# rakhimovv/lvt

Measured on AMD Instinct MI355X. Metric: video-clips/sec/node (VQVAE+DSFVT train step, BAIR 64x64x16), higher is better.
Workload: dtype f32

## Files before the change

### include/lvt_hip.h

```cpp
#ifndef LVT_HIP_H
#define LVT_HIP_H
#include <stddef.h>
#include <stdint.h>
#ifdef __cplusplus
extern "C" {
#endif

#define LVT_OK            0
#define LVT_EINVAL      (-1)
#define LVT_EWORKSPACE  (-2)
#define LVT_ELAUNCH     (-3)
#define LVT_ENODEVICE   (-4)

const char *lvt_last_error(void);
int lvt_version(void);
int lvt_device_info(char *name, int name_len, int *cus, int *clock_khz, long long *hbm_bytes);

#define LVT_MATH_F32   (1 << 16)
#define LVT_MATH_F16X2 (1 << 18)
typedef struct { const float *a; const float *b; float *c; } lvt_amax_io;
int lvt_amax(const float *x, long long n, float *out, void *stream);
typedef struct { const float *x; long long n; float *out; } lvt_amax_entry;
int lvt_amax_multi(const lvt_amax_entry *entries, int n, void *stream);
int lvt_amax_merge(const float *a, const float *b, float *out, void *stream);
// ... 23 lines not shown
    const float *B; long long ldb; int b_kb; long long b_skb;
    float *C;       long long ldc;
    int batch_outer, batch_inner;
    long long sA_o, sA_i, sB_o, sB_i, sC_o, sC_i;
    float alpha;
    int flags;
    const float *bias;
    const float *res;  long long ldr;
    const float *mask; long long ldm;
    int splits;
    float *a_colsum;
    long long c_plane;
    const float *a_amax, *b_amax;
    const float *a_amax2, *b_amax2;
    float *c_amax;
} lvt_gemm_desc;
size_t lvt_gemm_workspace_bytes(const lvt_gemm_desc *d);
int lvt_gemm_f32(const lvt_gemm_desc *d, void *workspace, size_t workspace_bytes, void *stream);

int lvt_vq_argmax_scores(const float *scores, long long rows, int K, long long ld, const float *codebook, int D,
                         long long *idx, void *stream);

typedef struct {
    int M, N, K;
    const void *A; long long lda; int a_planes; int a_kb; long long a_skb;
    const void *B; long long ldb;
    float *C; long long ldc;
    int batch_outer, batch_inner;
    long long sA_o, sA_i, sB_o, sB_i, sC_o, sC_i;
    float alpha;
// ... 113 lines not shown
                     const float *g2_dev, const float *G, float *out, float *out_amax, void *stream);
int lvt_l1_bwd_plus(const float *a, const float *b, long long n, double denom, float scale, const float *gout_dev,
                    const float *g2_dev, const float *G, float *out, float *out_amax, void *stream);
int lvt_tanh_bwd(const float *g, const float *y, long long n, float *out, float *out_amax, void *stream);
int lvt_sigmoid_bwd(const float *g, const float *y, long long n, float *out, float *out_amax, void *stream);
int lvt_axpy(const float *x, const float *add, long long n, const float *alpha_dev, float alpha,
             float *out, void *stream);
int lvt_add_periodic(float *x, const float *table, long long rows, int P, int d, void *stream);

int lvt_layernorm_fwd(const float *x, long long rows, int d, float eps, const float *w, const float *b,
                      float *y, float *mean, float *rstd, float *y_amax, const float *w_amax, const float *b_amax,
                      void *stream);
int lvt_layernorm_fwd_p2(const float *x, long long rows, int d, float eps, const float *w, const float *b,
                         float *y, void *yp, float *mean, float *rstd, float *y_amax, const float *w_amax,
                         const float *b_amax, void *stream);
size_t lvt_layernorm_bwd_workspace_bytes(int d);
int lvt_layernorm_bwd(const float *dy, const float *x, const float *mean, const float *rstd,
                      const float *w, long long rows, int d, const float *add, float *dx, float *dw,
                      float *db, float *dx_amax, void *workspace, size_t workspace_bytes, void *stream);

int lvt_attn_softmax_fwd(float *scores, int B, int H, int S, float temper, const float *dt,
                         const float *dh, const float *dw, int bt, int bh, int bw, int masked, float fill,
                         void *stream);
int lvt_attn_softmax_bwd(const float *P, float *dP, int B, int H, int S, float temper, int bt, int bh,
                         int bw, float *G, float *ddt, float *ddh, float *ddw, void *stream);

int lvt_attn_fwd(const float *q, const float *k, const float *v, int B, int H, int S, int da, float temper,
                 const float *dt, const float *dh, const float *dw, int bt, int bh, int bw, int masked, float fill,
                 float *P, float *o, void *stream);

// ... 154 lines not shown
```

### lvt_amd/csrc/elementwise.hip

```cpp
#include "lvt_common.h"

static inline int grid_for(long long n, int per_block, int cap = 8192) {
    long long b = lvt_cdiv(n, per_block);
    if (b < 1) b = 1;
    return (int)(b < cap ? b : cap);
}

__device__ __forceinline__ float wave_sum(float v) {
#pragma unroll
    for (int off = 32; off >= 1; off >>= 1) v += __shfl_xor(v, off);
    return v;
}
__device__ __forceinline__ float wave_max(float v) {
#pragma unroll
    for (int off = 32; off >= 1; off >>= 1) v = fmaxf(v, __shfl_xor(v, off));
    return v;
}

__global__ void lvt_to_channels_last_kernel(const float *__restrict__ in, int B, int C, long long R, int ldo,
                                            int mode, const float *__restrict__ a, const float *__restrict__ s,
                                            float *__restrict__ out, float *__restrict__ out_amax) {
    __shared__ float amax_scratch[4];
    float am = 0.f;
    const long long total = (long long)B * R * ldo;
// ... 326 lines not shown
                const float a0 = v[i].x - mean, a1 = v[i].y - mean, a2 = v[i].z - mean, a3 = v[i].w - mean;
                q += (a0 * a0 + a1 * a1) + (a2 * a2 + a3 * a3);
            }
        }
        const float rstd = 1.0f / sqrtf(wave_sum(q) / d + eps);
        float4 *yp = reinterpret_cast<float4 *>(y + row * d);
#pragma unroll
        for (int i = 0; i < LN_MAXV; ++i) {
            const int c = lane + 64 * i;
            if (c < d4) {
                const float4 ww = reinterpret_cast<const float4 *>(w)[c];
                const float4 bb = reinterpret_cast<const float4 *>(b)[c];
                float4 o;
                o.x = (v[i].x - mean) * rstd * ww.x + bb.x; o.y = (v[i].y - mean) * rstd * ww.y + bb.y;
                o.z = (v[i].z - mean) * rstd * ww.z + bb.z; o.w = (v[i].w - mean) * rstd * ww.w + bb.w;
                yp[c] = o;
                if (P2) {
                    uint2 ph, pl;
                    ln_split_pair(o.x, o.y, ps, ph.x, pl.x);
                    ln_split_pair(o.z, o.w, ps, ph.y, pl.y);
                    char *ip = yimg + (long long)row * d * 4 + (c >> 3) * 128 + (c & 7) * 8;
                    *reinterpret_cast<uint2 *>(ip) = ph;
                    *reinterpret_cast<uint2 *>(ip + 64) = pl;
                }
                am = fmaxf(am, fmaxf(fmaxf(lvt_absf(o.x), lvt_absf(o.y)), fmaxf(lvt_absf(o.z), lvt_absf(o.w))));
            }
        }
        if (lane == 0 && mean_out) { mean_out[row] = mean; rstd_out[row] = rstd; }
    }
    if (y_amax) lvt_block_amax_commit(am, y_amax, amax_scratch);
}
// ... 5 lines not shown
    LVT_REQUIRE(!w_amax == !b_amax, "layernorm_fwd: w_amax and b_amax come together");
    hipLaunchKernelGGL(lvt_layernorm_fwd_kernel<0>, dim3(grid_for(rows, 4, (y_amax && !w_amax) ? 2048 : LN_FWD_MAX_BLOCKS)), dim3(256), 0,
                       (hipStream_t)stream, x, rows, d, eps, w, b, y, mean, rstd, y_amax, w_amax, b_amax, (char *)nullptr);
    LVT_CHECK_LAUNCH("lvt_layernorm_fwd_kernel");
    return LVT_OK;
}
extern "C" int lvt_layernorm_fwd_p2(const float *x, long long rows, int d, float eps, const float *w, const float *b,
                                    float *y, void *yp, float *mean, float *rstd, float *y_amax, const float *w_amax,
                                    const float *b_amax, void *stream) {
    LVT_REQUIRE(x && w && b && y && yp && rows > 0 && d % 32 == 0 && d <= 256 * LN_MAXV, "layernorm_fwd_p2: bad args (d=%d)", d);
    LVT_REQUIRE(y_amax && w_amax && b_amax, "layernorm_fwd_p2: the image is scaled by the a-priori bound: y_amax, w_amax, b_amax are required");
    LVT_REQUIRE(((uintptr_t)yp & 127) == 0, "layernorm_fwd_p2: the image must be 128-byte aligned");
    hipLaunchKernelGGL(lvt_layernorm_fwd_kernel<1>, dim3(grid_for(rows, 4, LN_FWD_MAX_BLOCKS)), dim3(256), 0,
                       (hipStream_t)stream, x, rows, d, eps, w, b, y, mean, rstd, y_amax, w_amax, b_amax, (char *)yp);
    LVT_CHECK_LAUNCH("lvt_layernorm_fwd_kernel<p2>");
    return LVT_OK;
}

#define LN_BWD_BLOCKS 512
#define LN_BWD_ROWS 1
__global__ __launch_bounds__(256) void lvt_layernorm_bwd_kernel(
    const float *__restrict__ dy, const float *__restrict__ x, const float *__restrict__ mean,
    const float *__restrict__ rstd, const float *__restrict__ w, long long rows, int d, const float *__restrict__ add,
    float *__restrict__ dx, float *__restrict__ pdw, float *__restrict__ pdb, float *__restrict__ dx_amax) {
    __shared__ float amax_scratch[4];
    float am = 0.f;
    __shared__ float sdw[4][256 * LN_MAXV];
    __shared__ float sdb[4][256 * LN_MAXV];
    const int lane = threadIdx.x & 63, wave = threadIdx.x >> 6;
    const int d4 = d / 4;
// ... 280 lines not shown
```

### lvt_amd/csrc/gemm_engine.hip

```cpp
#include "lvt_common.h"
#include "epilogue_fast.h"
#include <string.h>
#include <stdlib.h>
#include <stdint.h>
#include <type_traits>

typedef float f32x16 __attribute__((ext_vector_type(16)));

#define BK 32
#define NTHREADS 256

enum { A_KPLAIN = 0, A_MPLAIN = 1, A_CONV_K = 2, A_CONVT_K = 3, A_CONV_M = 4, A_ONEHOT_M = 5, A_PATCH = 6, A_PATCHT = 7 };
enum { B_KPLAIN = 0, B_NPLAIN = 1, B_CONVT_W = 2 };

struct KParams {
    int M, N, K;
    const float *A; long long lda; int a_kb; long long a_skb;
    const float *B; long long ldb; int b_kb; long long b_skb;
    float *C; long long ldc; long long c_plane;
    int batch_inner;
    long long sA_o, sA_i, sB_o, sB_i, sC_o, sC_i;
    float alpha; int flags;
    const float *bias; const float *res; long long ldr; const float *mask; long long ldm;
    int splits; int k_per_split; float *partial; long long partial_stride;
    int vec_epi;
    float *colsum_partial;
    const float *a_amax, *b_amax;
    const float *a_amax2, *b_amax2;
    float *c_amax;
    lvt_conv_geom g;
    const char *b_img;
    int Tq, Hq, Wq;
    int jT, jH, jW;
    const long long *oh_idx; long long oh_bstride, oh_pstride; int oh_P, oh_V; int oh_off[32];
};

__device__ __forceinline__ float4 ldg4(const float *p) { return *reinterpret_cast<const float4 *>(p); }

__device__ __forceinline__ unsigned cvt_pk_bf16(float lo, float hi) {
    unsigned r;
    asm("v_cvt_pk_bf16_f32 %0, %1, %2" : "=v"(r) : "v"(lo), "v"(hi));
    return r;
}
__device__ __forceinline__ float bf_lo(unsigned p) { return __uint_as_float(p << 16); }
// ... 1267 lines not shown
    else lvt_epilogue_vec<A_PATCHT, BM, BN, WM, WN>(p, acc, lds, m0, n0, wm, wn, lane, phase, 0, 0, 0);
}

#define WIDE_THREADS 512
#define WT_PA (256 + 32)
#define WT_PB (128 + 32)
typedef short s16x4 __attribute__((ext_vector_type(4)));
__device__ __forceinline__ f16x8 wide_tr_frag(const unsigned short *p, int pitch4) {
    typedef __attribute__((address_space(3))) s16x4 lds_v4;
    const s16x4 lo = __builtin_amdgcn_ds_read_tr16_b64_v4i16((lds_v4 *)(p));
    const s16x4 hi = __builtin_amdgcn_ds_read_tr16_b64_v4i16((lds_v4 *)(p + pitch4));
    union { struct { s16x4 a, b; } s; f16x8 v; } u;
    u.s.a = lo; u.s.b = hi;
    return u.v;
}
template <int TA, int TB>
__global__ __launch_bounds__(WIDE_THREADS, 2) void lvt_gemm_wide_kernel(const KParams p) {
    constexpr int BM = 256, BN = 128, WM = 4, WN = 2, TM = 2, TN = 2;
    constexpr int AMODE = TA ? A_MPLAIN : A_KPLAIN;
    constexpr int PA = WT_PA, PB = WT_PB;
    constexpr int PSA = TA ? BK * PA : HPlane<BM>::SIZE, PSB = TB ? BK * PB : HPlane<BN>::SIZE;
    constexpr int STAGE = 2 * (PSA + PSB);
    static_assert(PA % 4 == 0 && PB % 4 == 0 && PSA % 8 == 0 && PSB % 8 == 0, "transposing reads need 8-byte aligned addresses");
    static_assert(BK * PA <= HPlane<BM>::SIZE && BK * PB <= HPlane<BN>::SIZE, "the memory-order images are the smaller ones");
    constexpr int STAGE_FLOATS = (2 * STAGE) / 2 + 8;
    constexpr int TURN_FLOATS = WM * WN * 32 * (TN * 32);
    constexpr int LDS_FLOATS = STAGE_FLOATS > TURN_FLOATS ? STAGE_FLOATS : TURN_FLOATS;
    __shared__ __attribute__((aligned(16))) float lds[LDS_FLOATS];
    unsigned short *S0 = reinterpret_cast<unsigned short *>(lds);

    const int tid = threadIdx.x, lane = tid & 63, wave = tid >> 6;
    const int wm = wave / WN, wn = wave % WN;
// ... 5 lines not shown
    const float sa = lvt_f16_scale(p.a_amax, unscale, p.a_amax2), sb = lvt_f16_scale(p.b_amax, unscale, p.b_amax2);

    float4 av[4], bv[2];
    const int r0 = tid >> 3, kq = tid & 7;
    const int kk0 = TA ? tid >> 6 : 0, mq = tid & 63;
    const int bkk0 = tid >> 5, bnq = tid & 31;
    const char *Ak = reinterpret_cast<const char *>(tc.A), *Bk = reinterpret_cast<const char *>(tc.B);
    unsigned aoff[4], boff_g[2];
    int a_kin = 0, b_kin = 0;
    if (!TA) {
#pragma unroll
        for (int i = 0; i < 4; ++i) aoff[i] = (unsigned)(((long long)min(m0 + r0 + 64 * i, p.M - 1) * p.lda + kq * 4) * 4);
        const int blk = kbeg / p.a_kb;
        a_kin = kbeg - blk * p.a_kb;
        Ak += ((long long)blk * p.a_skb + a_kin) * 4;
    } else {
        const int m = m0 + mq * 4;
#pragma unroll
        for (int i = 0; i < 4; ++i) aoff[i] = (unsigned)(((long long)(kk0 * 4 + i) * p.lda + (m < p.M ? m : 0)) * 4);
        Ak += (long long)kbeg * p.lda * 4;
    }
    if (!TB) {
#pragma unroll
        for (int i = 0; i < 2; ++i) boff_g[i] = (unsigned)(((long long)min(n0 + r0 + 64 * i, p.N - 1) * p.ldb + kq * 4) * 4);
        const int blk = kbeg / p.b_kb;
        b_kin = kbeg - blk * p.b_kb;
        Bk += ((long long)blk * p.b_skb + b_kin) * 4;
    } else {
        const int n = n0 + bnq * 4;
#pragma unroll
        for (int i = 0; i < 2; ++i) boff_g[i] = (unsigned)(((long long)(bkk0 * 2 + i) * p.ldb + (n < p.N ? n : 0)) * 4);
        Bk += (long long)kbeg * p.ldb * 4;
    }
    const bool sum_on = TA && p.colsum_partial != nullptr && n0 == 0;
    float4 colacc = zero4();
    auto fetch = [&]() {
#pragma unroll
        for (int i = 0; i < 4; ++i) av[i] = *reinterpret_cast<const float4 *>(Ak + aoff[i]);
        if (!TA) {
            a_kin += BK;
            const bool wrap = a_kin >= p.a_kb;
            Ak += wrap ? ((long long)p.a_skb - p.a_kb + BK) * 4 : (long long)BK * 4;
            a_kin = wrap ? 0 : a_kin;
        } else {
            Ak += (long long)BK * p.lda * 4;
            if (sum_on) {
#pragma unroll
                for (int i = 0; i < 4; ++i) { colacc.x += av[i].x; colacc.y += av[i].y; colacc.z += av[i].z; colacc.w += av[i].w; }
            }
// ... 4 lines not shown
            b_kin += BK;
            const bool wrap = b_kin >= p.b_kb;
            Bk += wrap ? ((long long)p.b_skb - p.b_kb + BK) * 4 : (long long)BK * 4;
            b_kin = wrap ? 0 : b_kin;
        } else {
#pragma unroll
            for (int i = 0; i < 2; ++i) bv[i] = *reinterpret_cast<const float4 *>(Bk + boff_g[i]);
            Bk += (long long)BK * p.ldb * 4;
        }
    };
    auto store = [&](unsigned short *buf) {
        unsigned short *Ah = buf, *Bh = buf + 2 * PSA;
        if (!TA) {
#pragma unroll
            for (int i = 0; i < 4; ++i) store_split2_k<BM>(Ah, r0 + 64 * i, kq * 4, av[i], sa);
        } else {
#pragma unroll
            for (int i = 0; i < 4; ++i) {
                uint2 ph, pl;
                split2(av[i], sa, ph, pl);
                unsigned short *d = Ah + (kk0 * 4 + i) * PA + mq * 4;
                *reinterpret_cast<uint2 *>(d) = ph;
                *reinterpret_cast<uint2 *>(d + PSA) = pl;
            }
        }
        if (!TB) {
#pragma unroll
            for (int i = 0; i < 2; ++i) store_split2_k<BN>(Bh, r0 + 64 * i, kq * 4, bv[i], sb);
        } else {
#pragma unroll
// ... 318 lines not shown
    }
    if ((p.flags & LVT_EPI_PLANES) && !pv.vec_epi) {
        lvt_set_error("gemm: LVT_EPI_PLANES needs 16-byte aligned bias / res / mask and ldr, ldm %% 4 == 0");
        return LVT_EINVAL;
    }
    if (math_of(p.flags) == 2)
        hipLaunchKernelGGL((lvt_gemm_kernel<AMODE, BMODE, BM, BN, WM, WN, 2>), grid, dim3(NTHREADS), 0, s, pv);
    else if (math_of(p.flags) == 1)
        hipLaunchKernelGGL((lvt_gemm_kernel<AMODE, BMODE, BM, BN, WM, WN, 1>), grid, dim3(NTHREADS), 0, s, pv);
    else
        hipLaunchKernelGGL((lvt_gemm_kernel<AMODE, BMODE, BM, BN, WM, WN, 0>), grid, dim3(NTHREADS), 0, s, pv);
    LVT_CHECK_LAUNCH("lvt_gemm_kernel");
    return LVT_OK;
}

template <int TA, int TB>
static int launch_wide(const KParams &p, int zcount, hipStream_t s) {
    const long long ntm = lvt_cdiv(p.M, 256), ntn = lvt_cdiv(p.N, 128);
    if (ntm * ntn > 0x7fffffffLL || zcount > 65535 || p.splits > 65535) {
        lvt_set_error("gemm: grid too large (%lld tiles, z=%d, splits=%d)", ntm * ntn, zcount, p.splits);
        return LVT_EINVAL;
    }
    dim3 grid((unsigned)(ntm * ntn), (unsigned)zcount, (unsigned)(p.splits > 1 ? p.splits : 1));
    KParams pv = p;
    {
        auto al16 = [](const void *q) { return ((uintptr_t)q & 15) == 0; };
        bool ok = p.N % 4 == 0;
        if (p.splits > 1) ok = ok && al16(p.partial) && p.partial_stride % 4 == 0 && ((long long)p.M * p.N) % 4 == 0;
        else {
            ok = ok && al16(p.C) && p.ldc % 4 == 0 && p.sC_o % 4 == 0 && p.sC_i % 4 == 0;
            if (p.flags & LVT_EPI_BIAS) ok = ok && al16(p.bias);
            if (p.flags & LVT_EPI_RESIDUAL) ok = ok && al16(p.res) && p.ldr % 4 == 0;
            if (p.flags & LVT_EPI_MASK) ok = ok && al16(p.mask) && p.ldm % 4 == 0;
        }
        pv.vec_epi = ok ? 1 : 0;
    }
    if ((p.flags & LVT_EPI_PLANES) && !pv.vec_epi) {
        lvt_set_error("gemm: LVT_EPI_PLANES needs 16-byte aligned bias / res / mask and ldr, ldm %% 4 == 0");
        return LVT_EINVAL;
    }
    hipLaunchKernelGGL((lvt_gemm_wide_kernel<TA, TB>), grid, dim3(WIDE_THREADS), 0, s, pv);
    LVT_CHECK_LAUNCH("lvt_gemm_wide_kernel");
    return LVT_OK;
}

static int choose_splits(long long tiles, int K, int min_k) {
    int s = (int)((2 * LVT_NUM_CU) / (tiles > 0 ? tiles : 1));
    const int maxs = K / min_k > 0 ? K / min_k : 1;
    if (s > maxs) s = maxs;
    if (s < 1) s = 1;
    return s;
}

static void kparams_from_desc(const lvt_gemm_desc *d, KParams &p) {
    memset(&p, 0, sizeof(p));
    p.M = d->M; p.N = d->N; p.K = d->K;
    p.A = d->A; p.lda = d->lda; p.a_kb = d->a_kb > 0 ? d->a_kb : d->K; p.a_skb = d->a_skb;
    p.B = d->B; p.ldb = d->ldb; p.b_kb = d->b_kb > 0 ? d->b_kb : d->K; p.b_skb = d->b_skb;
    p.C = d->C; p.ldc = d->ldc; p.c_plane = d->c_plane;
    p.batch_inner = d->batch_inner > 0 ? d->batch_inner : 1;
    p.sA_o = d->sA_o; p.sA_i = d->sA_i; p.sB_o = d->sB_o; p.sB_i = d->sB_i; p.sC_o = d->sC_o; p.sC_i = d->sC_i;
    p.alpha = d->alpha; p.flags = d->flags; p.bias = d->bias; p.res = d->res; p.ldr = d->ldr;
    p.mask = d->mask; p.ldm = d->ldm;
    p.splits = d->splits > 1 ? d->splits : 1;
    p.a_amax = d->a_amax; p.b_amax = d->b_amax; p.c_amax = d->c_amax;
    p.a_amax2 = d->a_amax2; p.b_amax2 = d->b_amax2;
}

static int gemm_batch(const lvt_gemm_desc *d) {
    return (d->batch_outer > 0 ? d->batch_outer : 1) * (d->batch_inner > 0 ? d->batch_inner : 1);
}

extern "C" size_t lvt_gemm_workspace_bytes(const lvt_gemm_desc *d) {
    if (!d || d->splits <= 1) return 0;
    return (size_t)d->splits * gemm_batch(d) * ((size_t)d->M * d->N + (d->a_colsum ? (size_t)d->M : 0)) * sizeof(float);
}

extern "C" int lvt_gemm_f32(const lvt_gemm_desc *d, void *workspace, size_t workspace_bytes, void *stream) {
    LVT_REQUIRE(d && d->A && d->B && d->C, "gemm: null pointer");
    LVT_REQUIRE(d->M > 0 && d->N > 0 && d->K > 0, "gemm: bad shape %d %d %d", d->M, d->N, d->K);
    LVT_REQUIRE(d->K % 4 == 0, "gemm: K=%d must be a multiple of 4", d->K);
// ... 28 lines not shown
            return LVT_EWORKSPACE;
        }
        p.k_per_split = (int)(lvt_cdiv(lvt_cdiv(p.K, p.splits), BK) * BK);
        p.partial = (float *)workspace;
        p.partial_stride = (long long)zc * d->M * d->N;
        if (d->a_colsum) {
            LVT_REQUIRE(d->ta == 1 && d->M % 4 == 0, "gemm: a_colsum needs ta == 1 and M %% 4 == 0");
            p.colsum_partial = p.partial + (long long)p.splits * p.partial_stride;
        }
    } else {
        LVT_REQUIRE(!d->a_colsum, "gemm: a_colsum needs splits > 1");
    }
    int rc;
    const long long a_span = d->ta ? (long long)d->K * d->lda : (long long)d->M * d->lda + (long long)(d->K / p.a_kb) * d->a_skb;
    const long long b_span = d->tb ? (long long)d->K * d->ldb : (long long)d->N * d->ldb + (long long)(d->K / p.b_kb) * d->b_skb;
    const bool wide = math_of(d->flags) == 2 && d->M > 128 && d->K % BK == 0 && p.a_kb % BK == 0 &&
                      p.b_kb % BK == 0 && a_span < (1LL << 30) && b_span < (1LL << 30) &&
                      !(d->flags & (LVT_CAUSAL_KMAX | LVT_CAUSAL_KMIN | LVT_CAUSAL_TILE));
    if (wide && d->ta == 0 && d->tb == 0) rc = launch_wide<0, 0>(p, zc, s);
    else if (wide && d->ta == 0 && d->tb == 1) rc = launch_wide<0, 1>(p, zc, s);
    else if (wide) rc = launch_wide<1, 1>(p, zc, s);
    else if (d->ta == 0 && d->tb == 0) rc = launch_tile<A_KPLAIN, B_KPLAIN, 128, 128, 2, 2>(p, zc, s);
    else if (d->ta == 0 && d->tb == 1) rc = launch_tile<A_KPLAIN, B_NPLAIN, 128, 128, 2, 2>(p, zc, s);
    else rc = launch_tile<A_MPLAIN, B_NPLAIN, 128, 128, 2, 2>(p, zc, s);
    if (rc != LVT_OK) return rc;
    if (p.splits > 1) {
        const long long n4 = p.partial_stride / 4;
        const int blocks = (int)(lvt_cdiv(n4, 256) < 2048 ? lvt_cdiv(n4, 256) : 2048);
        hipLaunchKernelGGL(lvt_reduce_splits_kernel, dim3(blocks), dim3(256), 0, s, p.partial, n4,
                           p.partial_stride, p.splits, d->C, (d->flags & LVT_EPI_ACCUM) ? 1 : 0);
        LVT_CHECK_LAUNCH("lvt_reduce_splits_kernel");
        if (p.colsum_partial) {
            hipLaunchKernelGGL(lvt_reduce_splits_kernel, dim3((unsigned)lvt_cdiv((long long)zc * d->M / 4, 256)), dim3(256), 0, s,
                               (const float *)p.colsum_partial, (long long)zc * d->M / 4, (long long)zc * d->M, p.splits,
// ... 535 lines not shown
```

### lvt_amd/hip/binding.py

```python
import ctypes as C
import os

import torch

_HERE = os.path.dirname(os.path.abspath(__file__))
_LIB_PATH = os.environ.get("LVT_HIP_LIB") or os.path.join(os.path.dirname(_HERE), "liblvt_hip.so")

EPI_BIAS, EPI_RESIDUAL, EPI_RELU, EPI_TANH, EPI_MASK, EPI_ACCUM, EPI_PLANES = 1, 2, 4, 8, 16, 32, 64
EPI_SIGMOID = 128
EPI_LEAKY, EPI_LEAKY_MASK = 1 << 11, 1 << 12


def epi_pad(n):
    if not 0 <= n <= 3:
        raise ValueError("epi_pad: 0..3 pad channels, got %r" % (n,))
    return n << 24
CAUSAL_KMAX, CAUSAL_KMIN, CAUSAL_TILE = 1 << 8, 1 << 9, 1 << 10
ABI_VERSION = 680
MATH_F32 = 1 << 16
MATH_F16X2 = 1 << 18
ONEHOT_DENSE = 1 << 19
WGRAD_DB_OF_X = 1 << 20
CONV_WEIGHT_IMAGE = 1 << 21
BN_RUNNING, BN_UPDATE, BN_UNBIASED, BN_COUNT, BN_TRAIN = 1, 2, 4, 8, 16
# ... 5 lines not shown

class GemmDesc(C.Structure):
    _fields_ = [
        ("M", C.c_int), ("N", C.c_int), ("K", C.c_int), ("ta", C.c_int), ("tb", C.c_int),
        ("A", C.c_void_p), ("lda", C.c_longlong), ("a_kb", C.c_int), ("a_skb", C.c_longlong),
        ("B", C.c_void_p), ("ldb", C.c_longlong), ("b_kb", C.c_int), ("b_skb", C.c_longlong),
        ("C", C.c_void_p), ("ldc", C.c_longlong),
        ("batch_outer", C.c_int), ("batch_inner", C.c_int),
        ("sA_o", C.c_longlong), ("sA_i", C.c_longlong), ("sB_o", C.c_longlong), ("sB_i", C.c_longlong),
        ("sC_o", C.c_longlong), ("sC_i", C.c_longlong),
        ("alpha", C.c_float), ("flags", C.c_int),
        ("bias", C.c_void_p), ("res", C.c_void_p), ("ldr", C.c_longlong),
        ("mask", C.c_void_p), ("ldm", C.c_longlong), ("splits", C.c_int),
        ("a_colsum", C.c_void_p), ("c_plane", C.c_longlong),
        ("a_amax", C.c_void_p), ("b_amax", C.c_void_p), ("a_amax2", C.c_void_p), ("b_amax2", C.c_void_p), ("c_amax", C.c_void_p),
    ]


class GemmP2Desc(C.Structure):
    _fields_ = [
        ("M", C.c_int), ("N", C.c_int), ("K", C.c_int),
        ("A", C.c_void_p), ("lda", C.c_longlong), ("a_planes", C.c_int), ("a_kb", C.c_int), ("a_skb", C.c_longlong),
        ("B", C.c_void_p), ("ldb", C.c_longlong),
        ("C", C.c_void_p), ("ldc", C.c_longlong),
        ("batch_outer", C.c_int), ("batch_inner", C.c_int),
        ("sA_o", C.c_longlong), ("sA_i", C.c_longlong), ("sB_o", C.c_longlong), ("sB_i", C.c_longlong),
        ("sC_o", C.c_longlong), ("sC_i", C.c_longlong),
        ("alpha", C.c_float), ("flags", C.c_int),
        ("bias", C.c_void_p), ("res", C.c_void_p), ("ldr", C.c_longlong),
        ("mask", C.c_void_p), ("ldm", C.c_longlong),
# ... 56 lines not shown


def _declare(lib):
    vp, ci, cll, cf, sz = C.c_void_p, C.c_int, C.c_longlong, C.c_float, C.c_size_t
    P = C.POINTER
    sigs = {
        "lvt_last_error": (C.c_char_p, []),
        "lvt_version": (ci, []),
        "lvt_device_info": (ci, [C.c_char_p, ci, P(ci), P(ci), P(cll)]),
        "lvt_gemm_workspace_bytes": (sz, [P(GemmDesc)]),
        "lvt_gemm_f32": (ci, [P(GemmDesc), vp, sz, vp]),
        "lvt_vq_argmax_scores": (ci, [vp, cll, ci, cll, vp, ci, vp, vp]),
        "lvt_gemm_p2_f32": (ci, [P(GemmP2Desc), vp]),
        "lvt_p2_pack_multi": (ci, [P(P2PackEntry), ci, vp]),
        "lvt_layernorm_fwd_p2": (ci, [vp, cll, ci, cf, vp, vp, vp, vp, vp, vp, vp, vp, vp, vp]),
        "lvt_gemm_smallm_f32": (ci, [ci, ci, ci, ci, vp, cll, vp, cll, vp, cll, ci, cll, cll, cf, ci, vp, vp, cll, vp, cll, cll, vp]),
        "lvt_gemm_smallm_splitk_workspace_bytes": (sz, [ci, ci, ci]),
        "lvt_gemm_smallm_splitk_f32": (ci, [ci, ci, ci, ci, vp, cll, vp, cll, vp, cll, cf, ci, vp, vp, cll, vp, cll, cll, vp, sz, vp]),
        "lvt_gemm_smallm_partial_f32": (ci, [ci, ci, ci, ci, vp, cll, vp, cll, vp, sz, vp]),
        "lvt_splitsum_layernorm_fwd": (ci, [vp, ci, ci, ci, vp, vp, cll, vp, cf, vp, vp, vp, vp]),
        "lvt_conv3d_pack_weight": (ci, [P(ConvGeom), vp, ci, ci, vp, vp]),
        "lvt_conv3d_pack_weight_t": (ci, [P(ConvGeom), vp, ci, ci, vp, vp]),
        "lvt_conv3d_uses_patch_kernel": (ci, [P(ConvGeom), ci]),
        "lvt_conv3d_fwd_uses_parity_kernel": (ci, [P(ConvGeom), ci]),
        "lvt_conv3d_pack_weight_parity": (ci, [P(ConvGeom), vp, ci, ci, vp, vp]),
        "lvt_amax": (ci, [vp, cll, vp, vp]),
        "lvt_amax_multi": (ci, [P(AmaxEntry), ci, vp]),
        "lvt_conv3d_pack_weights_multi": (ci, [P(PackEntry), ci, vp]),
        "lvt_conv3d_weight_image_bytes": (sz, [ci, ci]),
        "lvt_conv3d_weight_images": (ci, [P(WeightImageEntry), ci, vp]),
# ... 423 lines not shown
```

### lvt_amd/hip/ew.py

```python
import ctypes as C

import torch

from . import binding as L


def _f32(*shape, like):
    return torch.empty(*shape, dtype=torch.float32, device=like.device)


def to_channels_last(x_bcr, ldo, mode=0, a=None, s=None):
    L.require(x_bcr, a, s)
    B, Cc, R = x_bcr.shape
    out = _f32(B, R, ldo, like=x_bcr)
    L.check(L.lib().lvt_to_channels_last(L.ptr(x_bcr), B, Cc, R, ldo, mode, L.ptr(a), L.ptr(s), L.ptr(out),
                                         L.out_amax(out), L.stream_ptr()), "lvt_to_channels_last")
    return out


def to_channels_first(x_brc, Cc, mode=0, a=None, s=None, lo=0.0, hi=0.0):
    L.require(x_brc, a, s)
    B, R, ldi = x_brc.shape
    out = _f32(B, Cc, R, like=x_brc)
    L.check(L.lib().lvt_to_channels_first(L.ptr(x_brc), B, Cc, R, ldi, mode, L.ptr(a), L.ptr(s), lo, hi,
# ... 259 lines not shown


def layernorm_fwd_p2(x, w, b, eps=1e-5):
    L.require(x, w, b)
    d = x.shape[-1]
    rows = x.numel() // d
    y = torch.empty_like(x)
    yp = torch.empty_like(x)
    mean, rstd = _f32(rows, like=x), _f32(rows, like=x)
    L.check(L.lib().lvt_layernorm_fwd_p2(L.ptr(x), rows, d, eps, L.ptr(w), L.ptr(b), L.ptr(y), L.ptr(yp), L.ptr(mean),
                                         L.ptr(rstd), L.out_amax(y), L.ptr(L.amax_of(w)), L.ptr(L.amax_of(b)),
                                         L.stream_ptr()), "lvt_layernorm_fwd_p2")
    return y, yp, mean, rstd


def layernorm_bwd(dy, x, mean, rstd, w, add=None):
    L.require(dy, x, mean, rstd, w, add)
    d = x.shape[-1]
    rows = x.numel() // d
    dx = torch.empty_like(x)
    dw, db = _f32(d, like=x), _f32(d, like=x)
    n = L.lib().lvt_layernorm_bwd_workspace_bytes(d)
    ws = L.workspace(n, x.device, "ln")
    L.check(L.lib().lvt_layernorm_bwd(L.ptr(dy), L.ptr(x), L.ptr(mean), L.ptr(rstd), L.ptr(w), rows, d, L.ptr(add),
                                      L.ptr(dx), L.ptr(dw), L.ptr(db), L.out_amax(dx), L.ptr(ws), n, L.stream_ptr()),
            "lvt_layernorm_bwd")
    return dx, dw, db


def row_gather(x, perm, S):
# ... 9 lines not shown
```

### lvt_amd/hip/gemm.py

```python
import ctypes as C
import os

import torch

from . import binding as L


def gemm(A, B, C_out, M, N, K, ta=0, tb=0, lda=None, ldb=None, ldc=None, a_kb=0, a_skb=0, b_kb=0,
         b_skb=0, batch_outer=1, batch_inner=1, sA=(0, 0), sB=(0, 0), sC=(0, 0), alpha=1.0, flags=0,
         bias=None, res=None, ldr=0, mask=None, ldm=0, splits=1, a_colsum=None, c_plane=0, a_also=None, b_also=None):
    L.require(A, B, C_out, bias, res, mask)
    d = L.GemmDesc()
    d.M, d.N, d.K, d.ta, d.tb = M, N, K, ta, tb
    d.A, d.lda, d.a_kb, d.a_skb = A.data_ptr(), (lda if lda is not None else (K if ta == 0 else M)), a_kb, a_skb
    d.B, d.ldb, d.b_kb, d.b_skb = B.data_ptr(), (ldb if ldb is not None else (K if tb == 0 else N)), b_kb, b_skb
    d.C, d.ldc = C_out.data_ptr(), (ldc if ldc is not None else N)
    d.batch_outer, d.batch_inner = batch_outer, batch_inner
    d.sA_o, d.sA_i = sA
    d.sB_o, d.sB_i = sB
    d.sC_o, d.sC_i = sC
    d.alpha, d.flags = alpha, flags | L.math_flag()
    d.bias = bias.data_ptr() if bias is not None else None
    d.res = res.data_ptr() if res is not None else None
    d.ldr = ldr if res is not None and ldr else d.ldc
    d.mask = mask.data_ptr() if mask is not None else None
    d.ldm = ldm if mask is not None and ldm else d.ldc
    d.splits = splits
    d.a_colsum = a_colsum.data_ptr() if a_colsum is not None else None
    d.c_plane = c_plane
    if L.f16x2():
        d.a_amax, d.b_amax = L.amax_of(A).data_ptr(), L.amax_of(B).data_ptr()
        d.a_amax2 = L.amax_of(a_also).data_ptr() if a_also is not None else None
        d.b_amax2 = L.amax_of(b_also).data_ptr() if b_also is not None else None
        if splits <= 1 and C_out.dtype == torch.float32:
            d.c_amax = L.new_amax(C_out).data_ptr()
    if not d.c_amax:
        L.drop_amax(C_out)
    lib = L.lib()
    ws, nws = None, 0
    if splits > 1:
        nws = lib.lvt_gemm_workspace_bytes(C.byref(d))
        ws = L.workspace(nws, A.device, "gemm")
    t0 = L.TIMER.begin() if L.TIMER is not None else None
    L.check(lib.lvt_gemm_f32(C.byref(d), L.ptr(ws), nws, L.stream_ptr()), "lvt_gemm_f32")
    if t0 is not None:
        causal = 0.75 if flags & (L.CAUSAL_KMAX | L.CAUSAL_KMIN | L.CAUSAL_TILE) and M == 256 and N % 128 == 0 else 1.0
        L.TIMER.end("gemm_%s%s" % ("nt"[ta], "tn"[tb]), 2.0 * M * N * K * batch_outer * batch_inner * causal, t0)
    return C_out


class P2Image:
    __slots__ = ("data", "amax")

    def __init__(self, data, amax):
        self.data, self.amax = data, amax


def p2_mode(force=None):
    if not L.f16x2():
        return "off"
    if force is not None:
        return "full" if force else "off"
    env = os.environ.get("LVT_P2", "")
    if env == "qkv":
        return "qkv"
    return "full" if env not in ("", "0") else "off"


def p2_supported(force=None):
    return p2_mode(force) == "full"


def p2_pack(specs):
    arr = (L.P2PackEntry * len(specs))()
    for e, sp in zip(arr, specs):
        src, transpose, dst, amax = sp[:4]
        if src.dim() != 2 or dst.dim() != 2 or src.stride(1) != 1 or dst.stride(1) != 1 or not src.is_cuda:
            raise L.LvtError("p2_pack: 2-D device views with unit column stride expected")
        e.src, e.dst, e.rows, e.cols = src.data_ptr(), dst.data_ptr(), src.shape[0], src.shape[1]
        e.ld_src, e.ld_dst, e.transpose, e.amax = src.stride(0), dst.stride(0), int(bool(transpose)), amax.data_ptr()
        e.batch, e.bs_src, e.bs_dst = sp[4:7] if len(sp) > 4 else (1, 0, 0)
# ... 339 lines not shown
```

### lvt_amd/modeling/autoregressive/vt_attention.py

```python
import math
import os

import numpy as np
import torch
from torch import nn
from torch.nn import init

from ...hip import binding as L
from ...hip import dropout as D
from ...hip import ew, tx
from ...hip import gemm as G


class PositionalEncoding(nn.Module):

    def __init__(self, d_model, num_dims=3, min_timescale=1.0, max_timescale=1.0e4):
        super().__init__()
        assert d_model >= num_dims * 2, "d_model should be >= then 2*num_dims"
        self.d_model, self.num_dims = d_model, num_dims
        self.num_timescales = d_model // (num_dims * 2)
        inc = np.log(max_timescale / min_timescale) / self.num_timescales
        self.register_buffer("inv_timescales",
                             min_timescale * torch.exp(torch.arange(self.num_timescales).float() * -inc))
        self._tables = {}
# ... 79 lines not shown
        buf = getattr(m, "_p2_buf", None)
        if buf is None or buf[0].device != wqkv.device or buf[0].shape != (3 * na * da, d) or buf[1].shape != f1.weight.shape:
            buf = m._p2_buf = (torch.empty(3 * na * da, d, dtype=torch.float32, device=wqkv.device),
                               torch.empty_like(f1.weight, dtype=torch.float32))
        aq = L.amax_of(wqkv)
        specs.append((wqkv.view(3 * na * d, da)[:d], True, buf[0][:da], aq, 3 * na, d * da, da * d))
        i1 = None
        if full:
            a1 = L.amax_of(f1.weight)
            specs.append((f1.weight.detach(), False, buf[1], a1))
            i1 = G.P2Image(buf[1], a1)
        layers.append((m, G.P2Image(buf[0], aq), i1))
    if specs:
        G.p2_pack(specs)
    for m, iq, i1 in layers:
        m._p2 = (iq, i1)


def linear_wgrad(dy, x, n_out, k_in, rows, want_bias=False):
    dw = torch.empty(n_out, k_in, dtype=torch.float32, device=dy.device)
    tiles = -(-n_out // 128) * -(-k_in // 128)
    splits = _splits(tiles, rows)
    if not want_bias:
        G.gemm(dy, x, dw, n_out, k_in, rows, ta=1, tb=1, lda=dy.shape[-1], ldb=x.shape[-1], splits=splits)
        return dw
    if splits < 2:
        G.gemm(dy, x, dw, n_out, k_in, rows, ta=1, tb=1, lda=dy.shape[-1], ldb=x.shape[-1], splits=splits)
        return dw, G.colsum(dy, rows, n_out)
    db = torch.empty(n_out, dtype=torch.float32, device=dy.device)
    G.gemm(dy, x, dw, n_out, k_in, rows, ta=1, tb=1, lda=dy.shape[-1], ldb=x.shape[-1], splits=splits, a_colsum=db)
    return dw, db
# ... 40 lines not shown
class _BlockLocalAttentionFn(torch.autograd.Function):
    @staticmethod
    def forward(ctx, x, block, masked, dt, dh, dw, ln_w, ln_b, w_q, w_k, w_v, proj_w, f0w, f0b, f1w, f1b, f3w, f3b,
                wqkv, p2=None, drop=None):
        L.require(x)
        M, d = x.shape
        S = block[0] * block[1] * block[2]
        b = M // S
        na, _, da = w_q.shape
        hd = na * da
        temper = math.sqrt(da)
        dev = x.device
        flash = FUSED_ATTENTION and _use_flash(S, da, block, b * na)
        planes = FUSED_ATTENTION and not flash and _use_planes(S, da, block, b * na)
        p2 = p2 if (p2 is not None and not planes and L.f16x2()) else None
        p2_full = p2 is not None and p2[1] is not None
        if p2_full:
            xn, xn_img, mean1, rstd1 = ew.layernorm_fwd_p2(x, ln_w, ln_b)
        else:
            xn, mean1, rstd1 = ew.layernorm_fwd(x, ln_w, ln_b)
        if planes:
            qkv = torch.empty(3, 3, M, hd, dtype=torch.bfloat16, device=dev)
            G.gemm(xn, wqkv, qkv, M, da, d, ta=0, tb=1, lda=d, ldb=da, ldc=hd, batch_outer=3, batch_inner=na,
                   sB=(na * d * da, d * da), sC=(3 * M * hd, da), flags=L.EPI_PLANES, c_plane=M * hd)
            P, o = tx.attn_fwd_planes(qkv, b, na, S, da, temper, dt, dh, dw, block, masked)
        else:
            qkv = torch.empty(3, M, hd, dtype=torch.float32, device=dev)
            if p2 is not None:
                G.gemm_p2(G.P2Image(xn_img, L.amax_of(xn)) if p2_full else xn, p2[0], qkv, M, hd, d, lda=d, ldb=d, ldc=hd,
                          batch_outer=3, batch_inner=1, sB=(hd * d, 0), sC=(M * hd, 0))
                if p2_full:
                    del xn_img
            else:
                G.gemm(xn, wqkv, qkv, M, da, d, ta=0, tb=1, lda=d, ldb=da, ldc=hd, batch_outer=3, batch_inner=na,
                       sB=(na * d * da, d * da), sC=(M * hd, da))
            q, k, v = qkv[0], qkv[1], qkv[2]
        if planes:
            pass
        elif flash:
            o, P = tx.attn_fwd_flash(qkv, b, na, S, da, temper, dt, dh, dw, block, masked)
        elif FUSED_ATTENTION and tx.attn_fwd_supported(S, da):
            P, o = tx.attn_fwd(q, k, v, b, na, S, da, temper, dt, dh, dw, block, masked)
        else:
            P = torch.empty(b, na, S, S, dtype=torch.float32, device=dev)
            G.gemm(q, k, P, S, S, da, ta=0, tb=0, lda=hd, ldb=hd, ldc=S, batch_outer=b, batch_inner=na,
# ... 17 lines not shown
        else:
            fn, mean2, rstd2 = ew.layernorm_fwd(y1, f0w, f0b)
            G.gemm(fn, f1w, h1, M, f1w.shape[0], d, flags=L.EPI_BIAS | L.EPI_RELU, bias=f1b)
        if L.RELU_TRACE is not None:
            L.RELU_TRACE.append(h1 > 0)
        y2 = torch.empty(M, d, dtype=torch.float32, device=dev)
        if drop is None:
            G.gemm(h1, f3w, y2, M, d, f3w.shape[1], flags=L.EPI_BIAS | L.EPI_RESIDUAL, bias=f3b, res=y1)
        else:
            G.gemm(h1, f3w, y2, M, d, f3w.shape[1], flags=L.EPI_BIAS, bias=f3b)
            D.dropout_add(y2, y1, (seed, site + 1, pass_), p_drop, inplace=True)
        ctx.save_for_backward(x, mean1, rstd1, xn, qkv, P, o, y1, mean2, rstd2, fn, h1,
                              ln_w, wqkv, proj_w, f0w, f1w, f3w, dt, dh, dw)
        ctx.block, ctx.dims, ctx.masked, ctx.planes, ctx.flash = block, (M, d, S, b, na, da), bool(masked), bool(planes), bool(flash)
        ctx.drop = drop
        return y2

    @staticmethod
    def backward(ctx, dy2):
        (x, mean1, rstd1, xn, qkv, P, o, y1, mean2, rstd2, fn, h1,
         ln_w, wqkv, proj_w, f0w, f1w, f3w, dt, dh, dw) = ctx.saved_tensors
        M, d, S, b, na, da = ctx.dims
        hd = na * da
        temper = math.sqrt(da)
        dev = x.device
        dy2 = dy2.contiguous()
        dff = f1w.shape[0]
        drop = ctx.drop
        dz2 = dy2 if drop is None else D.dropout_bwd(dy2, (drop[1], drop[2] + 1, drop[3]), drop[0])
        dh1 = torch.empty(M, dff, dtype=torch.float32, device=dev)
# ... 39 lines not shown
        G.gemm(dP, q, dk, S, da, S, ta=1, tb=1, lda=S, ldb=hd, ldc=hd, sA=(na * S * S, S * S), sB=(S * hd, da),
               sC=(S * hd, da), flags=L.CAUSAL_KMIN if ctx.masked else 0, **bh)
        del dP
        return _BlockLocalAttentionFn._finish_backward(ctx, dqkv, ddt, ddh, ddw, dy1, dproj, df0w, df0b, df1w, df1b, df3w, df3b)

    @staticmethod
    def _finish_backward(ctx, dqkv, ddt, ddh, ddw, dy1, dproj, df0w, df0b, df1w, df1b, df3w, df3b):
        x, mean1, rstd1, xn = ctx.saved_tensors[:4]
        ln_w, wqkv = ctx.saved_tensors[12], ctx.saved_tensors[13]
        M, d, S, b, na, da = ctx.dims
        hd = na * da
        dev = x.device
        dxn = torch.empty(M, d, dtype=torch.float32, device=dev)
        G.gemm(dqkv, wqkv, dxn, M, d, 3 * hd, ta=0, tb=0, lda=hd, a_kb=hd, a_skb=M * hd, ldb=da, b_kb=da, b_skb=d * da)
        dws = torch.empty(3, na, d, da, dtype=torch.float32, device=dev)
        G.gemm(xn, dqkv, dws, d, da, M, ta=1, tb=1, lda=d, ldb=hd, ldc=da, batch_outer=3, batch_inner=na,
               sB=(M * hd, da), sC=(na * d * da, d * da), splits=_splits(3 * na * -(-d // 128), M))
        dx, dlnw, dlnb = ew.layernorm_bwd(dxn, x, mean1, rstd1, ln_w, add=dy1)
        return (dx, None, None, ddt, ddh, ddw, dlnw, dlnb, dws[0], dws[1], dws[2], dproj, df0w, df0b,
                df1w, df1b, df3w, df3b, None, None, None)


class BlockLocalAttention(nn.Module):
    def __init__(self, block_size, da, d, n_head, masked=False, dropout=0.0):
        super().__init__()
        self.block_size = tuple(block_size)
        self.n_head, self.masked = n_head, masked
        self.dropout = D.check_rate(dropout)
        self.bind_dropout(D.DropoutState(), 0)
        self.mha = MultiHeadAttention(n_head, d, da)
        self.ffn = nn.Sequential(nn.LayerNorm(d), nn.Linear(d, d), nn.ReLU(True), nn.Linear(d, d))
        t, h, w = self.block_size
# ... 85 lines not shown
```

Baseline: 1451.

## Keep layernorm output only as f16x2 image and consume it in both GEMMs

Adds an 'image' layernorm forward variant that writes only the pre-split f16 pair image of the normalized activations, scaled by an a-priori bound, instead of the fp32 output. The QKV projection GEMM and the weight-gradient GEMM in backward read this image directly through a new a_image path in the wide GEMM kernel. This path becomes the default P2 mode. It is meant to drop the fp32 xn store and re-splitting in the GEMMs, at the cost of new alignment constraints and no column-sum support.

```diff
diff --git a/include/lvt_hip.h b/include/lvt_hip.h
--- a/include/lvt_hip.h
+++ b/include/lvt_hip.h
@@ -61,6 +61,7 @@
     const float *a_amax, *b_amax;
     const float *a_amax2, *b_amax2;
     float *c_amax;
+    int a_image;
 } lvt_gemm_desc;
 size_t lvt_gemm_workspace_bytes(const lvt_gemm_desc *d);
 int lvt_gemm_f32(const lvt_gemm_desc *d, void *workspace, size_t workspace_bytes, void *stream);
@@ -204,6 +205,9 @@
 int lvt_layernorm_fwd_p2(const float *x, long long rows, int d, float eps, const float *w, const float *b,
                          float *y, void *yp, float *mean, float *rstd, float *y_amax, const float *w_amax,
                          const float *b_amax, void *stream);
+int lvt_layernorm_fwd_image(const float *x, long long rows, int d, float eps, const float *w, const float *b,
+                            void *yp, float *mean, float *rstd, float *y_amax, const float *w_amax,
+                            const float *b_amax, void *stream);
 size_t lvt_layernorm_bwd_workspace_bytes(int d);
 int lvt_layernorm_bwd(const float *dy, const float *x, const float *mean, const float *rstd,
                       const float *w, long long rows, int d, const float *add, float *dx, float *dw,
diff --git a/lvt_amd/csrc/elementwise.hip b/lvt_amd/csrc/elementwise.hip
--- a/lvt_amd/csrc/elementwise.hip
+++ b/lvt_amd/csrc/elementwise.hip
@@ -364,7 +364,7 @@
                 float4 o;
                 o.x = (v[i].x - mean) * rstd * ww.x + bb.x; o.y = (v[i].y - mean) * rstd * ww.y + bb.y;
                 o.z = (v[i].z - mean) * rstd * ww.z + bb.z; o.w = (v[i].w - mean) * rstd * ww.w + bb.w;
-                yp[c] = o;
+                if (P2 != 2) yp[c] = o;
                 if (P2) {
                     uint2 ph, pl;
                     ln_split_pair(o.x, o.y, ps, ph.x, pl.x);
@@ -400,6 +400,18 @@
     hipLaunchKernelGGL(lvt_layernorm_fwd_kernel<1>, dim3(grid_for(rows, 4, LN_FWD_MAX_BLOCKS)), dim3(256), 0,
                        (hipStream_t)stream, x, rows, d, eps, w, b, y, mean, rstd, y_amax, w_amax, b_amax, (char *)yp);
     LVT_CHECK_LAUNCH("lvt_layernorm_fwd_kernel<p2>");
+    return LVT_OK;
+}
+extern "C" int lvt_layernorm_fwd_image(const float *x, long long rows, int d, float eps, const float *w, const float *b,
+                                       void *yp, float *mean, float *rstd, float *y_amax, const float *w_amax,
+                                       const float *b_amax, void *stream) {
+    LVT_REQUIRE(x && w && b && yp && rows > 0 && d % 32 == 0 && d <= 256 * LN_MAXV, "layernorm_fwd_image: bad args (d=%d)", d);
+    LVT_REQUIRE(!mean == !rstd, "layernorm_fwd_image: mean and rstd come together");
+    LVT_REQUIRE(y_amax && w_amax && b_amax, "layernorm_fwd_image: the image is scaled by the a-priori bound: y_amax, w_amax, b_amax are required");
+    LVT_REQUIRE(((uintptr_t)yp & 127) == 0, "layernorm_fwd_image: the image must be 128-byte aligned");
+    hipLaunchKernelGGL(lvt_layernorm_fwd_kernel<2>, dim3(grid_for(rows, 4, LN_FWD_MAX_BLOCKS)), dim3(256), 0,
+                       (hipStream_t)stream, x, rows, d, eps, w, b, (float *)nullptr, mean, rstd, y_amax, w_amax, b_amax, (char *)yp);
+    LVT_CHECK_LAUNCH("lvt_layernorm_fwd_kernel<image>");
     return LVT_OK;
 }
 
diff --git a/lvt_amd/csrc/gemm_engine.hip b/lvt_amd/csrc/gemm_engine.hip
--- a/lvt_amd/csrc/gemm_engine.hip
+++ b/lvt_amd/csrc/gemm_engine.hip
@@ -28,6 +28,7 @@
     const float *a_amax, *b_amax;
     const float *a_amax2, *b_amax2;
     float *c_amax;
+    int a_image;
     lvt_conv_geom g;
     const char *b_img;
     int Tq, Hq, Wq;
@@ -1325,8 +1326,9 @@
     u.s.a = lo; u.s.b = hi;
     return u.v;
 }
-template <int TA, int TB>
+template <int TA, int TB, int AIMG = 0>
 __global__ __launch_bounds__(WIDE_THREADS, 2) void lvt_gemm_wide_kernel(const KParams p) {
+    static_assert(!AIMG || TA, "only the m-contiguous A operand has an image form");
     constexpr int BM = 256, BN = 128, WM = 4, WN = 2, TM = 2, TN = 2;
     constexpr int AMODE = TA ? A_MPLAIN : A_KPLAIN;
     constexpr int PA = WT_PA, PB = WT_PB;
@@ -1362,6 +1364,12 @@
         const int blk = kbeg / p.a_kb;
         a_kin = kbeg - blk * p.a_kb;
         Ak += ((long long)blk * p.a_skb + a_kin) * 4;
+    } else if (AIMG) {
+        const int m = m0 + ((lane >> 2) & 7) * 32;
+#pragma unroll
+        for (int i = 0; i < 4; ++i)
+            aoff[i] = (unsigned)(((long long)(wave + 8 * i) * p.lda + (m < p.M ? m : 0)) * 4 + (lane >> 5) * 64 + (lane & 3) * 16);
+        Ak += (long long)kbeg * p.lda * 4;
     } else {
         const int m = m0 + mq * 4;
 #pragma unroll
@@ -1380,7 +1388,7 @@
         for (int i = 0; i < 2; ++i) boff_g[i] = (unsigned)(((long long)(bkk0 * 2 + i) * p.ldb + (n < p.N ? n : 0)) * 4);
         Bk += (long long)kbeg * p.ldb * 4;
     }
-    const bool sum_on = TA && p.colsum_partial != nullptr && n0 == 0;
+    const bool sum_on = TA && !AIMG && p.colsum_partial != nullptr && n0 == 0;
     float4 colacc = zero4();
     auto fetch = [&]() {
 #pragma unroll
@@ -1415,6 +1423,12 @@
         if (!TA) {
 #pragma unroll
             for (int i = 0; i < 4; ++i) store_split2_k<BM>(Ah, r0 + 64 * i, kq * 4, av[i], sa);
+        } else if (AIMG) {
+            unsigned short *d = Ah + (lane >> 5) * PSA + wave * PA + (lane & 31) * 8;
+#pragma unroll
+            for (int i = 0; i < 4; ++i)
+                *reinterpret_cast<uint4 *>(d + i * (8 * PA)) = make_uint4(__float_as_uint(av[i].x), __float_as_uint(av[i].y),
+                                                                          __float_as_uint(av[i].z), __float_as_uint(av[i].w));
         } else {
 #pragma unroll
             for (int i = 0; i < 4; ++i) {
@@ -1763,7 +1777,7 @@
     return LVT_OK;
 }
 
-template <int TA, int TB>
+template <int TA, int TB, int AIMG = 0>
 static int launch_wide(const KParams &p, int zcount, hipStream_t s) {
     const long long ntm = lvt_cdiv(p.M, 256), ntn = lvt_cdiv(p.N, 128);
     if (ntm * ntn > 0x7fffffffLL || zcount > 65535 || p.splits > 65535) {
@@ -1788,7 +1802,7 @@
         lvt_set_error("gemm: LVT_EPI_PLANES needs 16-byte aligned bias / res / mask and ldr, ldm %% 4 == 0");
         return LVT_EINVAL;
     }
-    hipLaunchKernelGGL((lvt_gemm_wide_kernel<TA, TB>), grid, dim3(WIDE_THREADS), 0, s, pv);
+    hipLaunchKernelGGL((lvt_gemm_wide_kernel<TA, TB, AIMG>), grid, dim3(WIDE_THREADS), 0, s, pv);
     LVT_CHECK_LAUNCH("lvt_gemm_wide_kernel");
     return LVT_OK;
 }
@@ -1814,6 +1828,7 @@
     p.splits = d->splits > 1 ? d->splits : 1;
     p.a_amax = d->a_amax; p.b_amax = d->b_amax; p.c_amax = d->c_amax;
     p.a_amax2 = d->a_amax2; p.b_amax2 = d->b_amax2;
+    p.a_image = d->a_image;
 }
 
 static int gemm_batch(const lvt_gemm_desc *d) {
@@ -1872,10 +1887,19 @@
     int rc;
     const long long a_span = d->ta ? (long long)d->K * d->lda : (long long)d->M * d->lda + (long long)(d->K / p.a_kb) * d->a_skb;
     const long long b_span = d->tb ? (long long)d->K * d->ldb : (long long)d->N * d->ldb + (long long)(d->K / p.b_kb) * d->b_skb;
-    const bool wide = math_of(d->flags) == 2 && d->M > 128 && d->K % BK == 0 && p.a_kb % BK == 0 &&
+    const bool wide = math_of(d->flags) == 2 && (d->M > 128 || d->a_image) && d->K % BK == 0 && p.a_kb % BK == 0 &&
                       p.b_kb % BK == 0 && a_span < (1LL << 30) && b_span < (1LL << 30) &&
                       !(d->flags & (LVT_CAUSAL_KMAX | LVT_CAUSAL_KMIN | LVT_CAUSAL_TILE));
-    if (wide && d->ta == 0 && d->tb == 0) rc = launch_wide<0, 0>(p, zc, s);
+    if (d->a_image) {
+        LVT_REQUIRE(math_of(d->flags) == 2, "gemm: a_image needs the f16x2 arithmetic (LVT_MATH_F16X2)");
+        LVT_REQUIRE(d->ta == 1 && d->tb == 1, "gemm: a_image is served in the (ta=1, tb=1) form only");
+        LVT_REQUIRE(!d->a_colsum, "gemm: a_image cannot produce a_colsum (the column sums need the fp32 operand)");
+        LVT_REQUIRE(d->lda % 32 == 0 && d->K % 32 == 0, "gemm: a_image needs lda %% 32 == 0 and K %% 32 == 0 (lda=%lld, K=%d)", d->lda, d->K);
+        LVT_REQUIRE(((uintptr_t)d->A & 127) == 0 && d->sA_o % 32 == 0 && d->sA_i % 32 == 0 && !d->a_amax2,
+                    "gemm: a_image: A 128-byte aligned, batch strides %% 32 == 0, one scale (no a_amax2)");
+        LVT_REQUIRE(wide, "gemm: a_image: operand spans of 4 GB or more per batch and the causal forms are not served");
+        rc = launch_wide<1, 1, 1>(p, zc, s);
+    } else if (wide && d->ta == 0 && d->tb == 0) rc = launch_wide<0, 0>(p, zc, s);
     else if (wide && d->ta == 0 && d->tb == 1) rc = launch_wide<0, 1>(p, zc, s);
     else if (wide) rc = launch_wide<1, 1>(p, zc, s);
     else if (d->ta == 0 && d->tb == 0) rc = launch_tile<A_KPLAIN, B_KPLAIN, 128, 128, 2, 2>(p, zc, s);
diff --git a/lvt_amd/hip/binding.py b/lvt_amd/hip/binding.py
--- a/lvt_amd/hip/binding.py
+++ b/lvt_amd/hip/binding.py
@@ -43,6 +43,7 @@
         ("mask", C.c_void_p), ("ldm", C.c_longlong), ("splits", C.c_int),
         ("a_colsum", C.c_void_p), ("c_plane", C.c_longlong),
         ("a_amax", C.c_void_p), ("b_amax", C.c_void_p), ("a_amax2", C.c_void_p), ("b_amax2", C.c_void_p), ("c_amax", C.c_void_p),
+        ("a_image", C.c_int),
     ]
 
 
@@ -129,6 +130,7 @@
         "lvt_gemm_p2_f32": (ci, [P(GemmP2Desc), vp]),
         "lvt_p2_pack_multi": (ci, [P(P2PackEntry), ci, vp]),
         "lvt_layernorm_fwd_p2": (ci, [vp, cll, ci, cf, vp, vp, vp, vp, vp, vp, vp, vp, vp, vp]),
+        "lvt_layernorm_fwd_image": (ci, [vp, cll, ci, cf, vp, vp, vp, vp, vp, vp, vp, vp, vp]),
         "lvt_gemm_smallm_f32": (ci, [ci, ci, ci, ci, vp, cll, vp, cll, vp, cll, ci, cll, cll, cf, ci, vp, vp, cll, vp, cll, cll, vp]),
         "lvt_gemm_smallm_splitk_workspace_bytes": (sz, [ci, ci, ci]),
         "lvt_gemm_smallm_splitk_f32": (ci, [ci, ci, ci, ci, vp, cll, vp, cll, vp, cll, cf, ci, vp, vp, cll, vp, cll, cll, vp, sz, vp]),
diff --git a/lvt_amd/hip/ew.py b/lvt_amd/hip/ew.py
--- a/lvt_amd/hip/ew.py
+++ b/lvt_amd/hip/ew.py
@@ -297,6 +297,20 @@
     return y, yp, mean, rstd
 
 
+def layernorm_fwd_image(x, w, b, eps=1e-5):
+    from .gemm import P2Image
+    L.require(x, w, b)
+    d = x.shape[-1]
+    rows = x.numel() // d
+    yp = torch.empty_like(x)
+    mean, rstd = _f32(rows, like=x), _f32(rows, like=x)
+    bound = L.amax_slot(x.device)
+    L.check(L.lib().lvt_layernorm_fwd_image(L.ptr(x), rows, d, eps, L.ptr(w), L.ptr(b), L.ptr(yp), L.ptr(mean), L.ptr(rstd),
+                                            L.ptr(bound), L.ptr(L.amax_of(w)), L.ptr(L.amax_of(b)), L.stream_ptr()),
+            "lvt_layernorm_fwd_image")
+    return P2Image(yp, bound), mean, rstd
+
+
 def layernorm_bwd(dy, x, mean, rstd, w, add=None):
     L.require(dy, x, mean, rstd, w, add)
     d = x.shape[-1]
diff --git a/lvt_amd/hip/gemm.py b/lvt_amd/hip/gemm.py
--- a/lvt_amd/hip/gemm.py
+++ b/lvt_amd/hip/gemm.py
@@ -8,7 +8,12 @@
 
 def gemm(A, B, C_out, M, N, K, ta=0, tb=0, lda=None, ldb=None, ldc=None, a_kb=0, a_skb=0, b_kb=0,
          b_skb=0, batch_outer=1, batch_inner=1, sA=(0, 0), sB=(0, 0), sC=(0, 0), alpha=1.0, flags=0,
-         bias=None, res=None, ldr=0, mask=None, ldm=0, splits=1, a_colsum=None, c_plane=0, a_also=None, b_also=None):
+         bias=None, res=None, ldr=0, mask=None, ldm=0, splits=1, a_colsum=None, c_plane=0, a_also=None, b_also=None,
+         a_image=None):
+    if a_image is not None:
+        if a_also is not None:
+            raise L.LvtError("gemm: an A operand that spans two tensors (a_also) has no image form")
+        A = a_image.data
     L.require(A, B, C_out, bias, res, mask)
     d = L.GemmDesc()
     d.M, d.N, d.K, d.ta, d.tb = M, N, K, ta, tb
@@ -28,8 +33,10 @@
     d.splits = splits
     d.a_colsum = a_colsum.data_ptr() if a_colsum is not None else None
     d.c_plane = c_plane
+    d.a_image = int(a_image is not None)
     if L.f16x2():
-        d.a_amax, d.b_amax = L.amax_of(A).data_ptr(), L.amax_of(B).data_ptr()
+        d.a_amax = (a_image.amax if a_image is not None else L.amax_of(A)).data_ptr()
+        d.b_amax = L.amax_of(B).data_ptr()
         d.a_amax2 = L.amax_of(a_also).data_ptr() if a_also is not None else None
         d.b_amax2 = L.amax_of(b_also).data_ptr() if b_also is not None else None
         if splits <= 1 and C_out.dtype == torch.float32:
@@ -56,15 +63,22 @@
         self.data, self.amax = data, amax
 
 
+P2_DEFAULT = "xn"
+
+
 def p2_mode(force=None):
     if not L.f16x2():
         return "off"
     if force is not None:
         return "full" if force else "off"
     env = os.environ.get("LVT_P2", "")
+    if env == "":
+        return P2_DEFAULT
+    if env == "xn":
+        return "xn"
     if env == "qkv":
         return "qkv"
-    return "full" if env not in ("", "0") else "off"
+    return "full" if env != "0" else "off"
 
 
 def p2_supported(force=None):
diff --git a/lvt_amd/modeling/autoregressive/vt_attention.py b/lvt_amd/modeling/autoregressive/vt_attention.py
--- a/lvt_amd/modeling/autoregressive/vt_attention.py
+++ b/lvt_amd/modeling/autoregressive/vt_attention.py
@@ -117,7 +117,7 @@
     if specs:
         G.p2_pack(specs)
     for m, iq, i1 in layers:
-        m._p2 = (iq, i1)
+        m._p2 = (iq, i1, mode == "xn")
 
 
 def linear_wgrad(dy, x, n_out, k_in, rows, want_bias=False):
@@ -188,8 +188,15 @@
         flash = FUSED_ATTENTION and _use_flash(S, da, block, b * na)
         planes = FUSED_ATTENTION and not flash and _use_planes(S, da, block, b * na)
         p2 = p2 if (p2 is not None and not planes and L.f16x2()) else None
+        if p2 is not None and len(p2) > 2 and p2[2] and (M % 32 or d % 32 or da % 32 or M * max(d, hd) >= 1 << 30):
+            p2 = None
+        p2_xn = p2 is not None and len(p2) > 2 and bool(p2[2])
         p2_full = p2 is not None and p2[1] is not None
-        if p2_full:
+        xn_im = None
+        if p2_xn:
+            xn_im, mean1, rstd1 = ew.layernorm_fwd_image(x, ln_w, ln_b)
+            xn = xn_im.data
+        elif p2_full:
             xn, xn_img, mean1, rstd1 = ew.layernorm_fwd_p2(x, ln_w, ln_b)
         else:
             xn, mean1, rstd1 = ew.layernorm_fwd(x, ln_w, ln_b)
@@ -201,8 +208,10 @@
         else:
             qkv = torch.empty(3, M, hd, dtype=torch.float32, device=dev)
             if p2 is not None:
-                G.gemm_p2(G.P2Image(xn_img, L.amax_of(xn)) if p2_full else xn, p2[0], qkv, M, hd, d, lda=d, ldb=d, ldc=hd,
+                a_op = xn_im if p2_xn else (G.P2Image(xn_img, L.amax_of(xn)) if p2_full else xn)
+                G.gemm_p2(a_op, p2[0], qkv, M, hd, d, lda=d, ldb=d, ldc=hd,
                           batch_outer=3, batch_inner=1, sB=(hd * d, 0), sC=(M * hd, 0))
+                del a_op
                 if p2_full:
                     del xn_img
             else:
@@ -250,6 +259,7 @@
                               ln_w, wqkv, proj_w, f0w, f1w, f3w, dt, dh, dw)
         ctx.block, ctx.dims, ctx.masked, ctx.planes, ctx.flash = block, (M, d, S, b, na, da), bool(masked), bool(planes), bool(flash)
         ctx.drop = drop
+        ctx.xn_bound = xn_im.amax if p2_xn else None
         return y2
 
     @staticmethod
@@ -319,8 +329,9 @@
         dxn = torch.empty(M, d, dtype=torch.float32, device=dev)
         G.gemm(dqkv, wqkv, dxn, M, d, 3 * hd, ta=0, tb=0, lda=hd, a_kb=hd, a_skb=M * hd, ldb=da, b_kb=da, b_skb=d * da)
         dws = torch.empty(3, na, d, da, dtype=torch.float32, device=dev)
+        xn_im = G.P2Image(xn, ctx.xn_bound) if ctx.xn_bound is not None else None
         G.gemm(xn, dqkv, dws, d, da, M, ta=1, tb=1, lda=d, ldb=hd, ldc=da, batch_outer=3, batch_inner=na,
-               sB=(M * hd, da), sC=(na * d * da, d * da), splits=_splits(3 * na * -(-d // 128), M))
+               sB=(M * hd, da), sC=(na * d * da, d * da), splits=_splits(3 * na * -(-d // 128), M), a_image=xn_im)
         dx, dlnw, dlnb = ew.layernorm_bwd(dxn, x, mean1, rstd1, ln_w, add=dy1)
         return (dx, None, None, ddt, ddh, ddw, dlnw, dlnb, dws[0], dws[1], dws[2], dproj, df0w, df0b,
                 df1w, df1b, df3w, df3b, None, None, None)
```

After: 1462 (median of 6 runs). Within noise of the previous version (+0.7%).
